# gmongaras/Stable-Diffusion-3-From-Scratch

Measured on AMD Instinct MI355X. Metric: train images/sec MMDiT-B 256^2 bf16, higher is better.
Workload: dtype bf16

## Files before the change

stable-diffusion-3-from-scratch_amd/_lib.py:

```python
import ctypes
import os
import re

_HERE = os.path.dirname(os.path.abspath(__file__))
def experiment(name: str, default: str) -> str:
    return os.environ.get(name, default) if os.environ.get("MMDIT_EXPERIMENTS") == "1" else default


LIB_PATH = os.environ.get("MMDIT_LIB") or os.path.join(_HERE, "libmmdit_hip.so")
HEADER_PATH = os.path.join(_HERE, "..", "include", "mmdit_hip.h")
HEADER_EXT_PATH = os.path.join(_HERE, "..", "include", "mmdit_hip_ext.h")

F32, BF16 = 0, 1
ACT_NONE, ACT_SILU, ACT_SWIGLU, ACT_SWIGLU_BWD = 0, 1, 2, 3
PREC_BF16, PREC_SPLIT = 0, 1
FP8 = 2

_vp, _i, _i64, _f, _d = ctypes.c_void_p, ctypes.c_int, ctypes.c_int64, ctypes.c_float, ctypes.c_double


class GemmArgs(ctypes.Structure):
    _fields_ = [
        ("A", _vp), ("a_dtype", _i), ("a_kmajor", _i), ("lda", _i64),
        ("B", _vp), ("b_dtype", _i), ("b_kmajor", _i), ("ldb", _i64),
        ("C", _vp), ("c_dtype", _i), ("ldc", _i64),
        ("M", _i), ("N", _i), ("K", _i),
# ... 22 lines not shown
class LnBwdProblem(ctypes.Structure):
    _fields_ = [("dout", ctypes.c_void_p), ("x", ctypes.c_void_p), ("mean", ctypes.c_void_p), ("rstd", ctypes.c_void_p), ("scale", ctypes.c_void_p),
                ("ld_mod", ctypes.c_int64), ("dres", ctypes.c_void_p), ("rows", ctypes.c_int), ("rows_per_batch", ctypes.c_int),
                ("dx", ctypes.c_void_p), ("dscale", ctypes.c_void_p), ("dshift", ctypes.c_void_p), ("ld_dmod", ctypes.c_int64),
                ("acc", ctypes.c_void_p), ("gate", ctypes.c_void_p), ("ld_gate", ctypes.c_int64), ("dacc", ctypes.c_void_p), ("dgate", ctypes.c_void_p),
                ("ld_dgate", ctypes.c_int64), ("dbias", ctypes.c_void_p), ("ld_dbias", ctypes.c_int64)]


class QkProblem(ctypes.Structure):
    _fields_ = [("qkv", ctypes.c_void_p), ("wq", ctypes.c_void_p), ("wk", ctypes.c_void_p), ("rope_cos", ctypes.c_void_p), ("rope_sin", ctypes.c_void_p),
                ("tokens", ctypes.c_int), ("tok0", ctypes.c_int), ("dqkv", ctypes.c_void_p), ("dwq", ctypes.c_void_p), ("dwk", ctypes.c_void_p)]


class MlpBwdProblem(ctypes.Structure):
    _fields_ = [("dh", ctypes.c_void_p), ("gu", ctypes.c_void_p), ("dgu", ctypes.c_void_p), ("rows", ctypes.c_int), ("dbias", ctypes.c_void_p)]


class QkEpilogue(ctypes.Structure):
    _fields_ = [("wq", _vp), ("wk", _vp), ("rope_cos", _vp), ("rope_sin", _vp), ("tokens", _i), ("tok0", _i)]


_SIGNATURES = {
    "mmdit_abi_version": ([], _i),
    "mmdit_struct_size": ([_i], _i),
    "mmdit_build_arch": ([], ctypes.c_char_p),
    "mmdit_gemm": ([ctypes.POINTER(GemmArgs), _vp], _i),
    "mmdit_gemm_grouped": ([ctypes.POINTER(GemmArgs), _i, _vp], _i),
    "mmdit_gemm_plan": ([ctypes.POINTER(GemmArgs), _i], _i),
    "mmdit_gemm_set_workspace": ([_vp, ctypes.c_longlong], _i),
    "mmdit_debug_occupy": ([_i, ctypes.c_longlong, _vp], _i),
# ... 39 lines not shown
    "mmdit_vae_softmax_rows": ([_vp, _i, _i, _i, ctypes.c_float, _vp, _vp], _i),
    "mmdit_vae_attn_fwd": ([_vp, _vp, _vp, _i, _i, _i, _i, _f, _vp, _vp], _i),
    "mmdit_patchify": ([_vp, _i, _i, _i, _i, _i, _vp, _i, _vp], _i),
    "mmdit_unpatchify": ([_vp, _i, _i, _i, _i, _i, _vp, _i, _vp], _i),
    "mmdit_time_embed_fwd": ([_vp, _vp, _vp, _i, _i, _vp, _i, _vp], _i),
    "mmdit_time_embed_bwd": ([_vp, _i, _vp, _vp, _vp, _i, _i, _vp, _vp], _i),
    "mmdit_grad_sumsq": ([_vp, _vp, _vp, _i, _vp, _vp], _i),
    "mmdit_clip_coef": ([_vp, _i, _vp, _f, _vp, _vp], _i),
    "mmdit_adamw_step": ([_vp, _vp, _vp, _i, _vp, _vp, _d, _d, _d, _d, _d, _vp], _i),
    "mmdit_adamw_step_dlr": ([_vp, _vp, _vp, _i, _vp, _vp, _vp, _d, _d, _d, _d, _vp], _i),
    "mmdit_cast_multi": ([_vp, _vp, _vp, _i, _vp], _i),
}
_EXT_SIGNATURES = {
    "mmdit_attn_fwd_e4m3": ([_vp, _vp, _vp, _i, _i, _i, _i, _f, _vp, _vp, _vp, _vp, _vp], _i),
}
ATTN_E4M3_KEY_TILE, ATTN_E4M3_QUERY_TILE = 64, 128
ADAMW_CHUNK = 65536
ABI_VERSION = 10
_STRUCTS = [("mmdit_gemm_args", GemmArgs), ("mmdit_ln_fwd_problem", LnFwdProblem), ("mmdit_ln_bwd_problem", LnBwdProblem),
            ("mmdit_qk_problem", QkProblem), ("mmdit_mlp_bwd_problem", MlpBwdProblem), ("mmdit_adamw_tensor", None), ("mmdit_cast_tensor", None), ("mmdit_qk_epilogue", QkEpilogue)]

_lib = None


def declared_symbols():
    with open(HEADER_PATH) as f:
        txt = f.read()
    return sorted(set(re.findall(r"\b(mmdit_[a-z0-9_]+)\s*\(", txt)) - {"mmdit_stream_t"})


def declared_ext_symbols():
    with open(HEADER_EXT_PATH) as f:
        txt = f.read()
    return sorted(set(re.findall(r"\b(mmdit_[a-z0-9_]+)\s*\(", txt)) - {"mmdit_stream_t"})


def lib():
    global _lib
    if _lib is None:
        if not os.path.exists(LIB_PATH):
            raise RuntimeError(
                f"{LIB_PATH} is missing: build it with `python __graft_entry__.py build` "
                "(hipcc --offload-arch=gfx950).  There is no PyTorch/CPU fallback for the MMDiT hot path.")
        try:
            import torch
            if torch.cuda.is_available():
                torch.cuda.init()
        except ImportError:
            pass
        L = ctypes.CDLL(LIB_PATH)
        for name, (argtypes, restype) in list(_SIGNATURES.items()) + list(_EXT_SIGNATURES.items()):
            fn = getattr(L, name)
            fn.argtypes = argtypes
            fn.restype = restype
        if L.mmdit_abi_version() != ABI_VERSION:
            raise RuntimeError(f"{LIB_PATH}: ABI version {L.mmdit_abi_version()}, this binding is written for {ABI_VERSION}: rebuild (python __graft_entry__.py build)")
        for which, (name, struct) in enumerate(_STRUCTS):
            if struct is not None and L.mmdit_struct_size(which) != ctypes.sizeof(struct):
                raise RuntimeError(f"{LIB_PATH}: sizeof({name}) = {L.mmdit_struct_size(which)}, the binding's ctypes mirror has {ctypes.sizeof(struct)} bytes")
        _lib = L
    return _lib


ERR_ARG, ERR_DTYPE, ERR_SHAPE = -1, -2, -3


# ... 5 lines not shown
```

stable-diffusion-3-from-scratch_amd/build.py:

```python
import hashlib
import os
import subprocess
import sys
from concurrent.futures import ThreadPoolExecutor

HERE = os.path.dirname(os.path.abspath(__file__))
CSRC = os.path.join(HERE, "csrc")
LIB = os.path.join(HERE, "libmmdit_hip.so")
HEADER = os.path.join(HERE, "..", "include", "mmdit_hip.h")
HEADER_EXT = os.path.join(HERE, "..", "include", "mmdit_hip_ext.h")
SOURCES = ["gemm.hip", "gemm_dma.hip", "gemm_lean.hip", "gemm8p.hip", "gemm8p_inf.hip", "rowops.hip", "attention.hip", "attention_e4m3.hip", "vae.hip", "vae_attn.hip", "optim.hip"]
HIPCC = os.environ.get("HIPCC", "/opt/rocm/bin/hipcc")
FLAGS = ["--offload-arch=gfx950", "-O3", "-std=c++17", "-fPIC"] + os.environ.get("MMDIT_EXTRA_HIPCC_FLAGS", "").split()
SOURCE_FLAGS = {"vae_attn.hip": ["-mllvm", "-amdgpu-mfma-vgpr-form=1"]}


def _sha(paths, extra=""):
    h = hashlib.sha256(extra.encode())
    for p in paths:
        with open(p, "rb") as f:
            h.update(os.path.basename(p).encode() + b"\0" + f.read() + b"\0")
    return h.hexdigest()


def _read(path):
    try:
        with open(path) as f:
            return f.read().strip()
    except OSError:
        return None


def source_hash(src):
    headers = sorted(os.path.join(CSRC, f) for f in os.listdir(CSRC) if f.endswith(".h")) + [HEADER, HEADER_EXT]
    if src == "gemm8p_inf.hip":
        headers.append(os.path.join(CSRC, "gemm8p.hip"))
    return _sha([os.path.join(CSRC, src)] + headers, " ".join([HIPCC] + FLAGS + SOURCE_FLAGS.get(src, [])))


def build(force: bool = False, verbose: bool = False) -> str:
    want = {src: source_hash(src) for src in SOURCES}

    def cc(src):
        obj = os.path.join(CSRC, src.replace(".hip", ".o"))
        if not force and os.path.exists(obj) and _read(obj + ".sha") == want[src]:
            return obj, False
        cmd = [HIPCC] + FLAGS + SOURCE_FLAGS.get(src, []) + ["-c", os.path.join(CSRC, src), "-o", obj]
        if verbose:
            print(" ".join(cmd), flush=True)
# ... 27 lines not shown
```

stable-diffusion-3-from-scratch_amd/csrc/rowops.hip:

```cpp
#include "common.h"
#include <float.h>

namespace {

constexpr float LN_EPS = 1e-5f;
constexpr float RMS_EPS = FLT_EPSILON;

__device__ __forceinline__ float bf16_round(float x) { return __builtin_bit_cast(float, pack_bf2(x, 0.f) << 16); }

template <int NITX, typename TO, typename TA, bool RES, bool MX = false>
__device__ __forceinline__ void ln_mod_fwd_body(int block, const float* __restrict__ x, const float* __restrict__ scale, const float* __restrict__ shift,
                                                int64_t ld_mod, int rows, int d, int rpb, TO* __restrict__ out,
                                                float* __restrict__ mean_o, float* __restrict__ rstd_o,
                                                const TA* __restrict__ acc, const float* __restrict__ gate, int64_t ld_gate, float* __restrict__ xo,
                                                unsigned char* __restrict__ mx_scales) {
  constexpr int NIT = NITX < 0 ? -NITX : NITX;
  constexpr bool EXACT = NITX < 0;
  const int lane = threadIdx.x & 63, row = block * 4 + (threadIdx.x >> 6);
  if (row >= rows) return;
  const int nch = d >> 2;
  const int b = row / rpb;
  const float* xr = x + (int64_t)row * d;
  float v[NIT][4];
  float s = 0.f;
// ... 865 lines not shown
  __syncthreads();
  if (rl == 0 && c < cols && dbias) dbias[(int64_t)blockIdx.y * cols + c] += sb[0][cl] + sb[1][cl] + sb[2][cl] + sb[3][cl];
}

template <typename TI, typename TO>
__global__ void cast_kernel(const TI* __restrict__ src, TO* __restrict__ dst, int64_t n) {
  const int64_t n8 = n >> 3;
  for (int64_t i = (int64_t)blockIdx.x * blockDim.x + threadIdx.x; i < n8; i += (int64_t)gridDim.x * blockDim.x) {
    float v[8];
    ld8(src + i * 8, v);
    st8(dst + i * 8, v);
  }
  if (blockIdx.x == 0 && threadIdx.x < (n & 7)) io<TO>::st(dst + n8 * 8 + threadIdx.x, io<TI>::ld(src + n8 * 8 + threadIdx.x));
}

template <typename TI, typename TO, bool TO_TOKENS>
__global__ void patch_kernel(const TI* __restrict__ src, TO* __restrict__ dst, int batch, int ch, int H, int W) {
  const int W2 = W >> 1, H2 = H >> 1;
  const int64_t total = (int64_t)batch * ch * H * W2;
  for (int64_t g = (int64_t)blockIdx.x * blockDim.x + threadIdx.x; g < total; g += (int64_t)gridDim.x * blockDim.x) {
    const int j = (int)(g % W2); int64_t r = g / W2;
    const int y = (int)(r % H); r /= H;
    const int c = (int)(r % ch); const int64_t b = r / ch;
    const int64_t img_off = ((b * ch + c) * H + y) * W + 2 * j;
    const int64_t tok_off = ((b * H2 + (y >> 1)) * W2 + j) * (int64_t)(ch * 4) + c * 4 + (y & 1) * 2;
    if (TO_TOKENS) { io<TO>::st(dst + tok_off, io<TI>::ld(src + img_off)); io<TO>::st(dst + tok_off + 1, io<TI>::ld(src + img_off + 1)); }
    else { io<TO>::st(dst + img_off, io<TI>::ld(src + tok_off)); io<TO>::st(dst + img_off + 1, io<TI>::ld(src + tok_off + 1)); }
  }
}

// ... 592 lines not shown
  else if (x_dtype == MMDIT_BF16) hipLaunchKernelGGL((fp8_quant_kernel<bf16_t>), grid, dim3(256), 0, s, (const bf16_t*)x, n / 8, amax, (uint2*)q_fp8, scale);
  else return MMDIT_ERR_DTYPE;
  return mmdit_launch_status();
}

extern "C" int mmdit_cast(const void* src, int src_dtype, void* dst, int dst_dtype, int64_t n, mmdit_stream_t stream) {
  MMDIT_CHECK_ARG(src && dst && n > 0);
  hipStream_t s = (hipStream_t)stream;
  dim3 grid(grid_cap(n / 8 + 1, 256));
  if (src_dtype == MMDIT_F32 && dst_dtype == MMDIT_BF16) hipLaunchKernelGGL((cast_kernel<float, bf16_t>), grid, dim3(256), 0, s, (const float*)src, (bf16_t*)dst, n);
  else if (src_dtype == MMDIT_BF16 && dst_dtype == MMDIT_F32) hipLaunchKernelGGL((cast_kernel<bf16_t, float>), grid, dim3(256), 0, s, (const bf16_t*)src, (float*)dst, n);
  else return MMDIT_ERR_DTYPE;
  return mmdit_launch_status();
}

template <bool TO_TOKENS>
static int patch_dispatch(const void* src, int sdt, void* dst, int ddt, int batch, int ch, int H, int W, mmdit_stream_t stream) {
  MMDIT_CHECK_ARG(src && dst && batch > 0 && ch > 0 && H > 0 && W > 0 && H % 2 == 0 && W % 2 == 0);
  hipStream_t s = (hipStream_t)stream;
  dim3 grid(grid_cap((int64_t)batch * ch * H * (W / 2), 256));
#define PK(TI, TO) hipLaunchKernelGGL((patch_kernel<TI, TO, TO_TOKENS>), grid, dim3(256), 0, s, (const TI*)src, (TO*)dst, batch, ch, H, W)
  if (sdt == MMDIT_F32 && ddt == MMDIT_F32) PK(float, float);
  else if (sdt == MMDIT_F32 && ddt == MMDIT_BF16) PK(float, bf16_t);
  else if (sdt == MMDIT_BF16 && ddt == MMDIT_BF16) PK(bf16_t, bf16_t);
  else if (sdt == MMDIT_BF16 && ddt == MMDIT_F32) PK(bf16_t, float);
  else return MMDIT_ERR_DTYPE;
#undef PK
  return mmdit_launch_status();
}
extern "C" int mmdit_patchify(const void* img, int img_dtype, int batch, int ch, int H, int W, void* tokens, int tok_dtype, mmdit_stream_t st) {
// ... 24 lines not shown
```

stable-diffusion-3-from-scratch_amd/engine.py:

```python
from types import SimpleNamespace as NS

import torch

from . import _lib, ops
from ._lib import ACT_SILU, PREC_BF16, PREC_SPLIT

F32 = torch.float32
BF16 = torch.bfloat16


class Mode:
    def __init__(self, fast: bool = True, fp8: bool = False, mx: bool = False):
        self.fast = fast
        self.fp8 = fp8
        self.mx = mx
        self.T = BF16 if fast else F32
        self.prec = PREC_BF16 if fast else PREC_SPLIT
        self.attn_mode = 0 if fast else 1
        self.attn_e4m3 = False
        self._q = {}

    def act(self, t):
        return t if t.dtype == self.T else ops.cast(t, self.T)

# ... 336 lines not shown
    else:
        C2 = Pending(sv.C1)
    if not lazy:
        X2, C2 = X2.value(), C2.value()
    return X2, C2, sv


_LN_PAIR = _lib.experiment("MMDIT_LN_PAIR", "1") != "0"
_MX_FUSE = _lib.experiment("MMDIT_MX_FUSE", "1") != "0"
_BATCH_WMOD = _lib.experiment("MMDIT_BATCH_WMOD", "1") != "0"
_QKV_FUSE = _lib.experiment("MMDIT_QKV_FUSE", "1") != "0"
_QKV_RAW = _lib.experiment("MMDIT_QKV_RAW", "0") == "1"
_QK_FUSE = _lib.experiment("MMDIT_ATTN_QK_FUSE", "1") != "0"
_FUSE_SWIGLU_BWD = _lib.experiment("MMDIT_FUSE_SWIGLU_BWD", "1") != "0"
_FUSE_GATE = _lib.experiment("MMDIT_FUSE_GATE", "1") != "0"


def _qk_bwd_two_pass(m, w, sv, g, dOx, dOc, dims, rope, dev):
    B, N, Mt, H, d = dims
    S = N + Mt
    if w.kv_merge:
        dQ, dK, dV = ops.attn_bwd(sv.Q, sv.K, sv.V, sv.Ox, sv.Oc, dOx, dOc, sv.lse, N, 64 ** -0.5, m.T, s_kv=S // 2)
        return ops.qk_norm_rope_bwd_merge_pair(dQ, dK, dV, (sv.qkv_x, w.wq_x, w.wk_x, rope[0], rope[1], N, 0, g.wq_x, g.wk_x),
                                               (sv.qkv_c, w.wq_c, w.wk_c, None, None, Mt, N, g.wq_c, g.wk_c), B, H, S, m.T)
    dQ, dK, dV = ops.attn_bwd(sv.Q, sv.K, sv.V, sv.Ox, sv.Oc, dOx, dOc, sv.lse, N, 64 ** -0.5, m.T)
    if _LN_PAIR and dev.type == "cuda":
        return ops.qk_norm_rope_bwd_pair(dQ, dK, dV, (sv.qkv_x, w.wq_x, w.wk_x, rope[0], rope[1], N, 0, g.wq_x, g.wk_x),
                                         (sv.qkv_c, w.wq_c, w.wk_c, None, None, Mt, N, g.wq_c, g.wk_c), B, H, S, m.T)
    dqkv_x = ops.qk_norm_rope_bwd(dQ, dK, dV, sv.qkv_x, w.wq_x, w.wk_x, rope[0], rope[1], B, N, H, S, 0, g.wq_x, g.wk_x, m.T)
    dqkv_c = ops.qk_norm_rope_bwd(dQ, dK, dV, sv.qkv_c, w.wq_c, w.wk_c, None, None, B, Mt, H, S, N, g.wq_c, g.wk_c, m.T)
# ... 4 lines not shown
    B, N, Mt, H, d = dims
    both = not w.last
    ms = _mod_views(sv.mod, d, w.last)
    g = NS(mlp_x=NS(), mlp_c=NS() if both else None)
    hx = sv.gu_x.shape[1]
    nb = 2 if both else 1
    shapes = [(nb * d,), (hx,), (64,), (64,), (64,), (64,)] + ([(sv.gu_c.shape[1],)] if both else []) + ([] if defer_cond else [(d,)])
    npar = len(shapes)
    shapes += [tuple(sv.mod.shape), (B, nb * d)]
    zs, small_arena = _zeros_views(shapes, dev, prefix=npar)
    st = NS(g=g, ms=ms, zs=zs, npar=npar, small_arena=small_arena, both=both)
    st.bdown, g.mlp_x.bup, g.wq_x, g.wk_x, g.wq_c, g.wk_c = zs[:6]
    if not defer_cond:
        g.by = zs[npar - 1]
    st.dmod, st.bpart = zs[npar], zs[npar + 1]
    g.mlp_x.bdown = st.bdown[:d]
    if both:
        g.mlp_c.bdown, g.mlp_c.bup = st.bdown[d:], zs[6]
    st.dms = _mod_views(st.dmod, d, w.last)
    st.req_x = (sv.acc_mx, ms.gate2x, st.dms.gate2x, st.bpart[:, :d])
    st.req_c = (sv.acc_mc, ms.gate2c, st.dms.gate2c, st.bpart[:, d:]) if both else None
    return st


def block_bwd(m, w, sv, dX2, dC2, dy_acc, dims, rope, defer_cond=False, st=None, dacc=None, nxt=None, defer_wmod=False):
    B, N, Mt, H, d = dims
    S, dev = N + Mt, dX2.device
    both = not w.last
    if st is None:
        st = block_bwd_begin(m, w, sv, dims, dev, defer_cond)
    g, ms, dms, bpart, bdown, dmod = st.g, st.ms, st.dms, st.bpart, st.bdown, st.dmod
    pending = []
    fuse = _FUSE_GATE

    def defer(ns, name, dY, Xa):
        pending.append((lambda o, ns=ns, name=name: setattr(ns, name, o), _wg(dY, Xa)))

    dacc_x = dacc[0] if dacc is not None else ops.gate_residual_bwd(dX2, sv.acc_mx, ms.gate2x, N, dms.gate2x, bpart[:, :d], m.T)
    probs = [dict(A=dacc_x, B=w.mlp_x.Wdown, b_kmajor=True, out_dtype=m.T)]
    if both:
        dacc_c = dacc[1] if dacc is not None else ops.gate_residual_bwd(dC2, sv.acc_mc, ms.gate2c, Mt, dms.gate2c, bpart[:, d:], m.T)
        probs.append(dict(A=dacc_c, B=w.mlp_c.Wdown, b_kmajor=True, out_dtype=m.T))
    ops.colsum(bpart, bdown)
    dgu = None
    if (_FUSE_SWIGLU_BWD and m.fast and dev.type == "cuda" and m.prec == PREC_BF16 and dacc_x.dtype == BF16 and sv.gu_x.dtype == BF16
            and not w.mlp_x.gelu and (not both or not w.mlp_c.gelu)):
        fp = [dict(A=dacc_x, B=w.mlp_x.Wdown, aux=sv.gu_x, dbias=g.mlp_x.bup, precision=m.prec)]
        if both:
            fp.append(dict(A=dacc_c, B=w.mlp_c.Wdown, aux=sv.gu_c, dbias=g.mlp_c.bup, precision=m.prec))
        dgu = ops.gemm_swiglu_bwd(fp)
    if dgu is None:
        dh = _group(m, probs)
    defer(g.mlp_x, "Wdown", dacc_x, sv.h_x)
    pair = both and _LN_PAIR and dev.type == "cuda" and w.mlp_x.hidden == w.mlp_c.hidden and w.mlp_x.gelu == w.mlp_c.gelu
    if dgu is not None:
        dgu_x, dgu_c = dgu[0], (dgu[1] if both else None)
    elif pair:
        dgu_x, dgu_c = ops.mlp_act_bwd_pair((dh[0], sv.gu_x, g.mlp_x.bup), (dh[1], sv.gu_c, g.mlp_c.bup), w.mlp_x.hidden, w.mlp_x.gelu)
# ... 44 lines not shown
    else:
        dqkv_x, dqkv_c = _qk_bwd_two_pass(m, w, sv, g, dOx, dOc, dims, rope, dev)
    dln1 = _group(m, [dict(A=dqkv_x, B=w.Wqkv_x, b_kmajor=True, out_dtype=m.T), dict(A=dqkv_c, B=w.Wqkv_c, b_kmajor=True, out_dtype=m.T)])
    defer(g, "Wqkv_x", dqkv_x, sv.ln1x)
    defer(g, "Wqkv_c", dqkv_c, sv.ln1c)
    nacc = None
    ax = dict(dout=dln1[0], x=sv.X, mean=sv.mu1x, rstd=sv.rs1x, scale=ms.scale1x, dres=dX1, rpb=N, dscale=dms.scale1x, dshift=dms.shift1x)
    ac = dict(dout=dln1[1], x=sv.C, mean=sv.mu1c, rstd=sv.rs1c, scale=ms.scale1c, dres=dC1, rpb=Mt, dscale=dms.scale1c, dshift=dms.shift1c)
    if nxt is not None and fuse:
        ax["gated"], ac["gated"] = nxt.req_x, nxt.req_c
        (dX, nax), (dC, nac) = _ln_bwd_pair(ax, ac)
        nacc = (nax, nac)
    else:
        dX, dC = _ln_bwd_pair(ax, ac)

    dmod_a = m.act(dmod)
    if defer_cond:
        if not defer_wmod:
            defer(g, "Wmod", dmod_a, sv.yp)
        dy_acc = dmod_a
    else:
        defer(g, "Wmod", dmod_a, sv.yp)
        dyp = _dgrad(m, dmod_a, w.Wmod, F32, **({"split_k": 16} if m.fast else {}))
        dpre = ops.silu_bwd(dyp, sv.pre, m.T, g.by)
        dy_acc = _dgrad(m, dpre, w.Wy, F32, residual=dy_acc)
        defer(g, "Wy", dpre, sv.y)

    wg_arena = _wgrad_flush(m, pending)
    g.arenas = [wg_arena, st.small_arena] if wg_arena is not None else None
    if nxt is not None:
        return dX, dC, dy_acc, g, nacc
# ... 48 lines not shown
        elif torch.is_tensor(v):
            out.append(v)
    return out


def _set_grad_tensors(g, new, pos=0):
    for k, v in list(vars(g).items()):
        if isinstance(v, NS):
            pos = _set_grad_tensors(v, new, pos)
        elif torch.is_tensor(v):
            setattr(g, k, new[pos])
            pos += 1
    return pos


def model_bwd(m, W, sv, dv, rope, on_grads=None):
    B, N, Mt, H, d = sv.dims
    _, Cin, Hh, Ww = sv.img
    dev = dv.device
    if dev.type == "cuda":
        ops.zero_pool_begin(dev)
    g = NS()
    pending = []

    def defer(name, dY, Xa):
        pending.append((lambda o, name=name: setattr(g, name, o), _wg(dY, Xa)))

    dZ = ops.patchify(dv.contiguous(), m.T)
    g.bout = ops.zeros(W.Wout.shape[0], dev)
    ops.colsum(dZ, g.bout)
    dlnf = _dgrad(m, dZ, W.Wout, m.T)
    defer("Wout", dZ, sv.lnf)
    dmodo = ops.zeros(sv.modo.shape, dev) if sv.modo.dtype == F32 else torch.zeros_like(sv.modo)
    nblk = len(W.blocks)
    sts = [None] * nblk
    sts[nblk - 1] = block_bwd_begin(m, W.blocks[-1], sv.blocks[-1], sv.dims, dev, defer_cond=True)
    dacc = None
    if _FUSE_GATE:
        dX, dax = ops.ln_modulate_bwd(dlnf, sv.Xf, sv.muf, sv.rsf, sv.modo[:, d:], None, N, dmodo[:, d:], dmodo[:, :d], gated=sts[-1].req_x)
        dacc = (dax, None)
    else:
        dX = ops.ln_modulate_bwd(dlnf, sv.Xf, sv.muf, sv.rsf, sv.modo[:, d:], None, N, dmodo[:, d:], dmodo[:, :d])
    dmodo_a = m.act(dmodo)
    dy_acc = _dgrad(m, dmodo_a, W.Wmod_out, F32, **({"split_k": 4} if m.fast else {}))
    defer("Wmod_out", dmodo_a, sv.y)

    dC = None
    g.blocks = [None] * nblk
    dmods = [None] * nblk
    yps = [None] * nblk
    batch_wmod = on_grads is None and _BATCH_WMOD
    for i in range(nblk - 1, -1, -1):
        if i > 0:
            sts[i - 1] = block_bwd_begin(m, W.blocks[i - 1], sv.blocks[i - 1], sv.dims, dev, defer_cond=True)
            dX, dC, dmods[i], g.blocks[i], dacc = block_bwd(m, W.blocks[i], sv.blocks[i], dX, dC, None, sv.dims, rope, defer_cond=True,
                                                            st=sts[i], dacc=dacc, nxt=sts[i - 1], defer_wmod=batch_wmod)
        else:
            dX, dC, dmods[i], g.blocks[i] = block_bwd(m, W.blocks[i], sv.blocks[i], dX, dC, None, sv.dims, rope, defer_cond=True, st=sts[i], dacc=dacc,
                                                      defer_wmod=batch_wmod)
        sts[i] = None
        yps[i] = sv.blocks[i].yp
        sv.blocks[i] = None
        if on_grads is not None:
            repl = on_grads(_grad_tensors(g.blocks[i]), _wg_streams.get(dev), g.blocks[i].arenas)
            if repl is not None:
                _set_grad_tensors(g.blocks[i], repl)

    dyp_all = ops.zeros((nblk * B, d), dev)
    by_all = ops.zeros((nblk, d), dev)
    for i0 in range(0, nblk, 12):
        _group(m, [dict(A=dmods[i], B=W.blocks[i].Wmod, b_kmajor=True, out=dyp_all[i * B:(i + 1) * B], **({"split_k": 4} if m.fast else {}))
                   for i in range(i0, min(nblk, i0 + 12))])
    dpre_all = ops.silu_bwd(dyp_all, sv.pre_all, m.T, by_all, rows_per_bias=B)
    dyc = torch.empty((nblk + 1, B, d), dtype=F32, device=dev)
    dyc[nblk].copy_(dy_acc)
    for i0 in range(0, nblk, 12):
        _group(m, [dict(A=dpre_all[i * B:(i + 1) * B], B=W.blocks[i].Wy, b_kmajor=True, out=dyc[i]) for i in range(i0, min(nblk, i0 + 12))])
    dy_acc = dyc.sum(0)
    late = []
    for i in range(nblk):
        g.blocks[i].by = by_all[i]
        pending.append((lambda o, i=i: setattr(g.blocks[i], "Wy", o), _wg(dpre_all[i * B:(i + 1) * B], sv.y)))
        late += [(i, "by"), (i, "Wy")]
        if batch_wmod:
            pending.append((lambda o, i=i: setattr(g.blocks[i], "Wmod", o), _wg(dmods[i], yps[i])))

    g.bpe = ops.zeros(d, dev)
    ops.colsum(dX, g.bpe)
    dX_a = m.act(dX)
    dX0 = _dgrad(m, dX_a, W.Wpe, m.T)
    defer("Wpe", dX_a, sv.X0)
    defer("Wpatch", dX0, sv.patches)

    dCv = dC.view(B, Mt, d)
    dc1 = m.act(dCv[:, :W.split].reshape(B * W.split, d))
    dc2 = m.act(dCv[:, W.split:].reshape(B * (Mt - W.split), d))
    dcn1, dcn2 = _group(m, [dict(A=dc1, B=W.Wc1, b_kmajor=True, out_dtype=m.T), dict(A=dc2, B=W.Wc2, b_kmajor=True, out_dtype=m.T)])
    defer("Wc1", dc1, sv.cn1)
    defer("Wc2", dc2, sv.cn2)
    g.wn1, g.wn2, g.s1, g.s2 = ops.text_rmsnorm_bwd(dcn1, dcn2, sv.c, W.wn1, W.wn2, W.s1, W.s2, W.split)

    dy_a = m.act(dy_acc)
    defer("Wcond", dy_a, sv.cp)
    dpe = _dgrad(m, dy_a, W.Wt, m.T)
    defer("Wt", dy_a, sv.pe)
    g.time_scale = ops.time_embed_bwd(dpe, sv.t, W.time_scale, W.denom)
    _wgrad_flush(m, pending)
    if on_grads is not None:
        keys = [k for k, v in vars(g).items() if torch.is_tensor(v)]
        repl = on_grads([getattr(g, k) for k in keys] + [getattr(g.blocks[i], n) for i, n in late], _wg_streams.get(dev))
        if repl is not None:
# ... 7 lines not shown
```

stable-diffusion-3-from-scratch_amd/model_trainer.py:

```python
import copy
import json
import math
import os
import time

import torch
import torch.distributed as dist
from torch import nn

from .helpers.multi_gpu_helpers import is_main_process
from .helpers.TimeSampler import TimeSampler
from .helpers.checkpoint_stream import CheckpointStreamer
from .helpers.wire_format import unpad_latents
from .optim import ClipAdamW
from .reducer import GradReducer, broadcast_parameters


def get_scheduler(optimizer, num_warmup_steps, num_training_steps, use_lr_scheduler):
    if use_lr_scheduler:
        def lr_lambda(step):
            if step < num_warmup_steps:
                return float(step) / float(max(1, num_warmup_steps))
            progress = float(step - num_warmup_steps) / float(max(1, num_training_steps - num_warmup_steps))
            return max(0.0, 0.5 * (1.0 + math.cos(math.pi * 0.5 * 2.0 * progress)))
# ... 300 lines not shown
        return loss

    def can_capture(self):
        if self.device.type != "cuda" or not self.hip_optimizer:
            return "needs hip_optimizer=True on a GPU"
        if self.ema_model_cpu is not None and self._ema_gpu is None:
            return "the EMA must live on the GPU (ema_on_gpu=True) or be off"
        if self.reducer.enabled and dist.get_backend(self.subgroup) != "nccl":
            return "the gradient collectives are captured with the step: backend nccl (RCCL) only"
        return None

    def capture_graph(self, step):
        why = self.can_capture()
        if why is not None:
            raise RuntimeError("capture_graph: " + why)
        from . import engine
        if engine._WG_OVERLAP:
            engine._WG_OVERLAP = False
        in_graph = isinstance(self.data_source, SyntheticData) and self.device_rng
        self._slots = None
        if not in_graph:
            self._slots = [tuple(x.to(self.device).clone() for x in self._draw()) for _ in range(self.accumulation_steps)]
        torch.cuda.synchronize(self.device)
        if self.reducer.enabled and self.device.type == "cuda":
            self.capture_handoff = "polled" if self._wait_for_watchdog() else "heuristic"
        self.optim.sync_lr(self.device)
        self.optim.prepare_capture()
        self._loss_out = torch.zeros((), dtype=torch.float32, device=self.device)
        g = torch.cuda.CUDAGraph(keep_graph=True) if self.keep_graph else torch.cuda.CUDAGraph()
        for gen in (self._gen, getattr(self.data_source, "g", None)) if in_graph else ():
            if gen is not None:
                g.register_generator_state(gen)
        self.optim.zero_grad()
        try:
            with torch.cuda.graph(g, capture_error_mode="thread_local" if self.reducer.enabled else "global"):
                loss = None
                for k in range(self.accumulation_steps):
                    l = self.micro_step(final=(k == self.accumulation_steps - 1), inputs=None if in_graph else self._slots[k])
                    loss = l if loss is None else loss + l
                self._hip_optimizer_step()
                if self.grad_scaler is not None:
                    self.grad_scaler.update()
# ... 317 lines not shown
```

stable-diffusion-3-from-scratch_amd/ops.py:

```python
import ctypes
import os

import torch

from . import _lib
from ._lib import ACT_NONE, ACT_SILU, ACT_SWIGLU, ACT_SWIGLU_BWD, BF16, F32, FP8, PREC_BF16, PREC_SPLIT, GemmArgs, check

_DT = {torch.float32: F32, torch.bfloat16: BF16, torch.float8_e4m3fn: FP8}

PROFILE = None
_ZERO_ALL = _lib.experiment("MMDIT_ZERO_ALL", "0") == "1"


class _ZeroPool:

    def __init__(self):
        self.buf, self.off, self.cap, self.need = None, 0, 0, 0

    def begin(self, device):
        self.cap = max(self.cap, self.need)
        self.need, self.off = 0, 0
        self.buf = torch.zeros(self.cap, dtype=torch.float32, device=device) if self.cap else None

    def take(self, numel, device):
# ... 671 lines not shown
    if v.dtype != torch.float32 or x0.dtype != eps.dtype or x0.numel() != n or eps.numel() != n or n % 8:
        raise RuntimeError("flow_loss: v fp32, x0 and eps of one dtype and v's size, numel % 8 == 0")
    loss = torch.empty((), dtype=torch.float32, device=v.device)
    part = torch.empty(256, dtype=torch.float32, device=v.device)
    dv = torch.empty(v.shape, dtype=torch.float32, device=v.device) if need_grad else None
    check(_lib.lib().mmdit_flow_loss(_p(_c(v)), _p(_c(x0)), _p(_c(eps)), _dt(x0), n, 1.0 / (n * accumulation_steps), _p(dv), _p(part), _p(loss), _s()), "mmdit_flow_loss")
    return loss, dv


def colsum(x, out):
    rows, cols = x.shape
    check(_lib.lib().mmdit_colsum(_p(x), _dt(x), rows, cols, x.stride(0), _p(out), _s()), "mmdit_colsum")
    return out


def patchify(img, out_dtype):
    batch, ch, H, W = img.shape
    tokens = torch.empty((batch * (H // 2) * (W // 2), ch * 4), dtype=out_dtype, device=img.device)
    check(_lib.lib().mmdit_patchify(_p(_c(img)), _dt(img), batch, ch, H, W, _p(tokens), _dt(tokens), _s()), "mmdit_patchify")
    return tokens


def unpatchify(tokens, batch, ch, H, W, out_dtype):
    img = torch.empty((batch, ch, H, W), dtype=out_dtype, device=tokens.device)
    check(_lib.lib().mmdit_unpatchify(_p(_c(tokens)), _dt(tokens), batch, ch, H, W, _p(img), _dt(img), _s()), "mmdit_unpatchify")
    return img


def time_embed_fwd(t, time_scale, denom, out_dtype):
    batch, dim = t.shape[0], denom.shape[0]
# ... 76 lines not shown
```

Before: 2349.

## Add grouped backward-finish kernel fusing column sums and bf16 casts

```diff
diff --git a/include/mmdit_hip_train.h b/include/mmdit_hip_train.h
--- /dev/null
+++ b/include/mmdit_hip_train.h
@@ -0,0 +1,28 @@
+#ifndef MMDIT_HIP_TRAIN_H
+#define MMDIT_HIP_TRAIN_H
+
+#include "mmdit_hip.h"
+
+#ifdef __cplusplus
+extern "C" {
+#endif
+
+#define MMDIT_FINISH_MAX_PROBLEMS 64
+#define MMDIT_FINISH_TABLE_BYTES 8192
+
+typedef struct {
+  const void* x;
+  int x_dtype;
+  int groups, rows, cols;
+  int64_t ld, group_stride;
+  float* sum_out;
+  void* cast_out;
+} mmdit_finish_problem;
+
+int mmdit_backward_finish(const mmdit_finish_problem* probs, int count, void* table_dev, void* staging_host, mmdit_stream_t stream);
+
+#ifdef __cplusplus
+}
+#endif
+
+#endif
diff --git a/stable-diffusion-3-from-scratch_amd/_lib.py b/stable-diffusion-3-from-scratch_amd/_lib.py
--- a/stable-diffusion-3-from-scratch_amd/_lib.py
+++ b/stable-diffusion-3-from-scratch_amd/_lib.py
@@ -10,6 +10,7 @@
 LIB_PATH = os.environ.get("MMDIT_LIB") or os.path.join(_HERE, "libmmdit_hip.so")
 HEADER_PATH = os.path.join(_HERE, "..", "include", "mmdit_hip.h")
 HEADER_EXT_PATH = os.path.join(_HERE, "..", "include", "mmdit_hip_ext.h")
+HEADER_TRAIN_PATH = os.path.join(_HERE, "..", "include", "mmdit_hip_train.h")
 
 F32, BF16 = 0, 1
 ACT_NONE, ACT_SILU, ACT_SWIGLU, ACT_SWIGLU_BWD = 0, 1, 2, 3
@@ -62,6 +63,11 @@
 
 class MlpBwdProblem(ctypes.Structure):
     _fields_ = [("dh", ctypes.c_void_p), ("gu", ctypes.c_void_p), ("dgu", ctypes.c_void_p), ("rows", ctypes.c_int), ("dbias", ctypes.c_void_p)]
+
+
+class FinishProblem(ctypes.Structure):
+    _fields_ = [("x", ctypes.c_void_p), ("x_dtype", ctypes.c_int), ("groups", ctypes.c_int), ("rows", ctypes.c_int), ("cols", ctypes.c_int),
+                ("ld", ctypes.c_int64), ("group_stride", ctypes.c_int64), ("sum_out", ctypes.c_void_p), ("cast_out", ctypes.c_void_p)]
 
 
 class QkEpilogue(ctypes.Structure):
@@ -131,6 +137,10 @@
 _EXT_SIGNATURES = {
     "mmdit_attn_fwd_e4m3": ([_vp, _vp, _vp, _i, _i, _i, _i, _f, _vp, _vp, _vp, _vp, _vp], _i),
 }
+_TRAIN_SIGNATURES = {
+    "mmdit_backward_finish": ([ctypes.POINTER(FinishProblem), _i, _vp, _vp, _vp], _i),
+}
+FINISH_MAX_PROBLEMS, FINISH_TABLE_BYTES = 64, 8192
 ATTN_E4M3_KEY_TILE, ATTN_E4M3_QUERY_TILE = 64, 128
 ADAMW_CHUNK = 65536
 ABI_VERSION = 10
@@ -148,6 +158,12 @@
 
 def declared_ext_symbols():
     with open(HEADER_EXT_PATH) as f:
+        txt = f.read()
+    return sorted(set(re.findall(r"\b(mmdit_[a-z0-9_]+)\s*\(", txt)) - {"mmdit_stream_t"})
+
+
+def declared_train_symbols():
+    with open(HEADER_TRAIN_PATH) as f:
         txt = f.read()
     return sorted(set(re.findall(r"\b(mmdit_[a-z0-9_]+)\s*\(", txt)) - {"mmdit_stream_t"})
 
@@ -166,7 +182,7 @@
         except ImportError:
             pass
         L = ctypes.CDLL(LIB_PATH)
-        for name, (argtypes, restype) in list(_SIGNATURES.items()) + list(_EXT_SIGNATURES.items()):
+        for name, (argtypes, restype) in list(_SIGNATURES.items()) + list(_EXT_SIGNATURES.items()) + list(_TRAIN_SIGNATURES.items()):
             fn = getattr(L, name)
             fn.argtypes = argtypes
             fn.restype = restype
diff --git a/stable-diffusion-3-from-scratch_amd/build.py b/stable-diffusion-3-from-scratch_amd/build.py
--- a/stable-diffusion-3-from-scratch_amd/build.py
+++ b/stable-diffusion-3-from-scratch_amd/build.py
@@ -9,6 +9,7 @@
 LIB = os.path.join(HERE, "libmmdit_hip.so")
 HEADER = os.path.join(HERE, "..", "include", "mmdit_hip.h")
 HEADER_EXT = os.path.join(HERE, "..", "include", "mmdit_hip_ext.h")
+HEADER_TRAIN = os.path.join(HERE, "..", "include", "mmdit_hip_train.h")
 SOURCES = ["gemm.hip", "gemm_dma.hip", "gemm_lean.hip", "gemm8p.hip", "gemm8p_inf.hip", "rowops.hip", "attention.hip", "attention_e4m3.hip", "vae.hip", "vae_attn.hip", "optim.hip"]
 HIPCC = os.environ.get("HIPCC", "/opt/rocm/bin/hipcc")
 FLAGS = ["--offload-arch=gfx950", "-O3", "-std=c++17", "-fPIC"] + os.environ.get("MMDIT_EXTRA_HIPCC_FLAGS", "").split()
@@ -32,7 +33,7 @@
 
 
 def source_hash(src):
-    headers = sorted(os.path.join(CSRC, f) for f in os.listdir(CSRC) if f.endswith(".h")) + [HEADER, HEADER_EXT]
+    headers = sorted(os.path.join(CSRC, f) for f in os.listdir(CSRC) if f.endswith(".h")) + [HEADER, HEADER_EXT, HEADER_TRAIN]
     if src == "gemm8p_inf.hip":
         headers.append(os.path.join(CSRC, "gemm8p.hip"))
     return _sha([os.path.join(CSRC, src)] + headers, " ".join([HIPCC] + FLAGS + SOURCE_FLAGS.get(src, [])))
diff --git a/stable-diffusion-3-from-scratch_amd/csrc/rowops.hip b/stable-diffusion-3-from-scratch_amd/csrc/rowops.hip
--- a/stable-diffusion-3-from-scratch_amd/csrc/rowops.hip
+++ b/stable-diffusion-3-from-scratch_amd/csrc/rowops.hip
@@ -1,5 +1,7 @@
 #include "common.h"
+#include "../../include/mmdit_hip_train.h"
 #include <float.h>
+#include <string.h>
 
 namespace {
 
@@ -903,6 +905,68 @@
   if (blockIdx.x == 0 && threadIdx.x < (n & 7)) io<TO>::st(dst + n8 * 8 + threadIdx.x, io<TI>::ld(src + n8 * 8 + threadIdx.x));
 }
 
+struct FinProb {
+  const void* x; float* out; bf16_t* y;
+  int64_t ld, gs;
+  int rows, cols, f32, lc;
+  int rpt, nslab, nchunk, wg0;
+};
+struct FinTable { int wg_end[MMDIT_FINISH_MAX_PROBLEMS]; FinProb p[MMDIT_FINISH_MAX_PROBLEMS]; };
+static_assert(sizeof(FinTable) <= MMDIT_FINISH_TABLE_BYTES, "the finish table must fit the buffers the header promises");
+
+template <typename T>
+__device__ __forceinline__ void finish_body(const FinProb& p, int local, float* sbuf ) {
+  const int lc = p.lc, c = 1 << lc, nrl = 256 >> lc;
+  const int tx = threadIdx.x & (c - 1), rl = threadIdx.x >> lc;
+  const int slab = local % p.nslab, rest = local / p.nslab, chunk = rest % p.nchunk, g = rest / p.nchunk;
+  const int col = ((slab << lc) + tx) * 8;
+  const int rbeg = chunk * nrl * p.rpt, rend = min(p.rows, rbeg + nrl * p.rpt);
+  float s[8];
+#pragma unroll
+  for (int e = 0; e < 8; e++) s[e] = 0.f;
+  if (col < p.cols) {
+    const T* xb = (const T*)p.x + (int64_t)g * p.gs + col;
+    bf16_t* yb = p.y ? p.y + (int64_t)g * p.rows * p.cols + col : nullptr;
+    for (int r0 = rbeg + rl; r0 < rend; r0 += 4 * nrl) {
+      float v[4][8];
+#pragma unroll
+      for (int k = 0; k < 4; k++) ld8(xb + (int64_t)min(r0 + k * nrl, rend - 1) * p.ld, v[k]);
+#pragma unroll
+      for (int k = 0; k < 4; k++) {
+        const int r = r0 + k * nrl;
+        if (r < rend) {
+#pragma unroll
+          for (int e = 0; e < 8; e++) s[e] += v[k][e];
+          if (yb) st8(yb + (int64_t)r * p.cols, v[k]);
+        }
+      }
+    }
+  }
+  if (p.out) {
+    const int w = c * 8;
+    st8(sbuf + rl * w + tx * 8, s);
+    __syncthreads();
+    for (int j = threadIdx.x; j < w; j += 256) {
+      const int cc = (slab << lc) * 8 + j;
+      if (cc < p.cols) {
+        float t = 0.f;
+        for (int q = 0; q < nrl; q++) t += sbuf[q * w + j];
+        atomicAdd(p.out + cc, t);
+      }
+    }
+  }
+}
+
+__global__ __launch_bounds__(256) void backward_finish_kernel(const FinTable* __restrict__ tab, int count) {
+  __shared__ float sbuf[2048];
+  const int bid = blockIdx.x;
+  int pi = 0;
+  while (pi < count - 1 && bid >= tab->wg_end[pi]) pi++;
+  const FinProb p = tab->p[pi];
+  if (p.f32) finish_body<float>(p, bid - p.wg0, sbuf);
+  else finish_body<bf16_t>(p, bid - p.wg0, sbuf);
+}
+
 template <typename TI, typename TO, bool TO_TOKENS>
 __global__ void patch_kernel(const TI* __restrict__ src, TO* __restrict__ dst, int batch, int ch, int H, int W) {
   const int W2 = W >> 1, H2 = H >> 1;
@@ -1525,6 +1589,40 @@
   return mmdit_launch_status();
 }
 
+extern "C" int mmdit_backward_finish(const mmdit_finish_problem* probs, int count, void* table_dev, void* staging_host, mmdit_stream_t stream) {
+  MMDIT_CHECK_ARG(probs && table_dev && staging_host && count >= 1 && count <= MMDIT_FINISH_MAX_PROBLEMS && (uintptr_t)table_dev % 16 == 0);
+  FinTable t;
+  memset(&t, 0, sizeof(t));
+  int64_t wg = 0;
+  for (int i = 0; i < count; i++) {
+    const mmdit_finish_problem& q = probs[i];
+    MMDIT_CHECK_ARG(q.x && (q.sum_out || q.cast_out) && q.groups > 0 && q.rows > 0 && q.cols > 0 && q.cols % 8 == 0 && q.ld >= q.cols && q.ld % 8 == 0 &&
+                    q.group_stride >= 0 && q.group_stride % 8 == 0);
+    MMDIT_CHECK_ARG((uintptr_t)q.x % 16 == 0 && (uintptr_t)q.sum_out % 16 == 0 && (uintptr_t)q.cast_out % 16 == 0);
+    if (q.x_dtype != MMDIT_F32 && q.x_dtype != MMDIT_BF16) return MMDIT_ERR_DTYPE;
+    const bool flat = q.groups == 1 || (q.group_stride == (int64_t)q.rows * q.ld && (int64_t)q.groups * q.rows <= (1 << 30));
+    const int groups = flat ? 1 : q.groups, rows = flat ? q.groups * q.rows : q.rows;
+    if (rows > (1 << 30)) return MMDIT_ERR_SHAPE;
+    const int cp = q.cols / 8;
+    int lc = 8;
+    while (lc > 0 && (int64_t)((cp + (1 << lc) - 1) >> lc << lc) * 100 > (int64_t)cp * 115) lc--;
+    const int nrl = 256 >> lc;
+    const int64_t bytes = (int64_t)q.groups * q.rows * q.cols * (q.x_dtype == MMDIT_F32 ? 4 : 2);
+    const int rpt = bytes >= (16ll << 20) ? 8 : 4;
+    const int nslab = (cp + (1 << lc) - 1) >> lc, nchunk = (rows + nrl * rpt - 1) / (nrl * rpt);
+    t.p[i] = FinProb{q.x, q.sum_out, (bf16_t*)q.cast_out, q.ld, q.group_stride, rows, q.cols, q.x_dtype == MMDIT_F32, lc, rpt, nslab, nchunk, (int)wg};
+    wg += (int64_t)groups * nchunk * nslab;
+    if (wg > (1ll << 30)) return MMDIT_ERR_SHAPE;
+    t.wg_end[i] = (int)wg;
+  }
+  hipStream_t s = (hipStream_t)stream;
+  memcpy(staging_host, &t, sizeof(t));
+  hipError_t e = hipMemcpyAsync(table_dev, staging_host, sizeof(t), hipMemcpyHostToDevice, s);
+  if (e != hipSuccess) return (int)e;
+  hipLaunchKernelGGL(backward_finish_kernel, dim3((unsigned)wg), dim3(256), 0, s, (const FinTable*)table_dev, count);
+  return mmdit_launch_status();
+}
+
 template <bool TO_TOKENS>
 static int patch_dispatch(const void* src, int sdt, void* dst, int ddt, int batch, int ch, int H, int W, mmdit_stream_t stream) {
   MMDIT_CHECK_ARG(src && dst && batch > 0 && ch > 0 && H > 0 && W > 0 && H % 2 == 0 && W % 2 == 0);
diff --git a/stable-diffusion-3-from-scratch_amd/engine.py b/stable-diffusion-3-from-scratch_amd/engine.py
--- a/stable-diffusion-3-from-scratch_amd/engine.py
+++ b/stable-diffusion-3-from-scratch_amd/engine.py
@@ -374,6 +374,8 @@
 _QK_FUSE = _lib.experiment("MMDIT_ATTN_QK_FUSE", "1") != "0"
 _FUSE_SWIGLU_BWD = _lib.experiment("MMDIT_FUSE_SWIGLU_BWD", "1") != "0"
 _FUSE_GATE = _lib.experiment("MMDIT_FUSE_GATE", "1") != "0"
+_FINISH_FOLD = _lib.experiment("MMDIT_FINISH_FOLD", "0") == "1"
+_BIAS_DIRECT = _lib.experiment("MMDIT_BIAS_DIRECT", "0") == "1"
 
 
 def _qk_bwd_two_pass(m, w, sv, g, dOx, dOc, dims, rope, dev):
@@ -408,6 +410,9 @@
     if not defer_cond:
         g.by = zs[npar - 1]
     st.dmod, st.bpart = zs[npar], zs[npar + 1]
+    st.direct = _BIAS_DIRECT and dev.type == "cuda"
+    if st.direct:
+        st.bpart = st.bdown.unsqueeze(0).expand(B, nb * d)
     g.mlp_x.bdown = st.bdown[:d]
     if both:
         g.mlp_c.bdown, g.mlp_c.bup = st.bdown[d:], zs[6]
@@ -417,9 +422,10 @@
     return st
 
 
-def block_bwd(m, w, sv, dX2, dC2, dy_acc, dims, rope, defer_cond=False, st=None, dacc=None, nxt=None, defer_wmod=False):
+def block_bwd(m, w, sv, dX2, dC2, dy_acc, dims, rope, defer_cond=False, st=None, dacc=None, nxt=None, defer_wmod=False, defer_finish=False):
     B, N, Mt, H, d = dims
     S, dev = N + Mt, dX2.device
+    assert not defer_finish or (defer_cond and defer_wmod and st is not None)
     both = not w.last
     if st is None:
         st = block_bwd_begin(m, w, sv, dims, dev, defer_cond)
@@ -435,7 +441,8 @@
     if both:
         dacc_c = dacc[1] if dacc is not None else ops.gate_residual_bwd(dC2, sv.acc_mc, ms.gate2c, Mt, dms.gate2c, bpart[:, d:], m.T)
         probs.append(dict(A=dacc_c, B=w.mlp_c.Wdown, b_kmajor=True, out_dtype=m.T))
-    ops.colsum(bpart, bdown)
+    if not defer_finish and not st.direct:
+        ops.colsum(bpart, bdown)
     dgu = None
     if (_FUSE_SWIGLU_BWD and m.fast and dev.type == "cuda" and m.prec == PREC_BF16 and dacc_x.dtype == BF16 and sv.gu_x.dtype == BF16
             and not w.mlp_x.gelu and (not both or not w.mlp_c.gelu)):
@@ -510,7 +517,7 @@
     else:
         dX, dC = _ln_bwd_pair(ax, ac)
 
-    dmod_a = m.act(dmod)
+    dmod_a = dmod if defer_finish else m.act(dmod)
     if defer_cond:
         if not defer_wmod:
             defer(g, "Wmod", dmod_a, sv.yp)
@@ -589,6 +596,10 @@
     return pos
 
 
+def finish_launches(nblk):
+    return 1 + (2 * nblk + 4 + _lib.FINISH_MAX_PROBLEMS - 1) // _lib.FINISH_MAX_PROBLEMS
+
+
 def model_bwd(m, W, sv, dv, rope, on_grads=None):
     B, N, Mt, H, d = sv.dims
     _, Cin, Hh, Ww = sv.img
@@ -603,7 +614,12 @@
 
     dZ = ops.patchify(dv.contiguous(), m.T)
     g.bout = ops.zeros(W.Wout.shape[0], dev)
-    ops.colsum(dZ, g.bout)
+    finish = m.fast and dev.type == "cuda" and m.T == BF16
+    fold = finish and _FINISH_FOLD
+    if finish:
+        ops.backward_finish([(dZ, g.bout, None)])
+    else:
+        ops.colsum(dZ, g.bout)
     dlnf = _dgrad(m, dZ, W.Wout, m.T)
     defer("Wout", dZ, sv.lnf)
     dmodo = ops.zeros(sv.modo.shape, dev) if sv.modo.dtype == F32 else torch.zeros_like(sv.modo)
@@ -616,23 +632,28 @@
         dacc = (dax, None)
     else:
         dX = ops.ln_modulate_bwd(dlnf, sv.Xf, sv.muf, sv.rsf, sv.modo[:, d:], None, N, dmodo[:, d:], dmodo[:, :d])
-    dmodo_a = m.act(dmodo)
-    dy_acc = _dgrad(m, dmodo_a, W.Wmod_out, F32, **({"split_k": 4} if m.fast else {}))
-    defer("Wmod_out", dmodo_a, sv.y)
+    if not fold:
+        dmodo_a = m.act(dmodo)
+        dy_acc = _dgrad(m, dmodo_a, W.Wmod_out, F32, **({"split_k": 4} if m.fast else {}))
+        defer("Wmod_out", dmodo_a, sv.y)
 
     dC = None
     g.blocks = [None] * nblk
     dmods = [None] * nblk
     yps = [None] * nblk
     batch_wmod = on_grads is None and _BATCH_WMOD
+    fin_blocks = fold and batch_wmod
+    fin = []
     for i in range(nblk - 1, -1, -1):
         if i > 0:
             sts[i - 1] = block_bwd_begin(m, W.blocks[i - 1], sv.blocks[i - 1], sv.dims, dev, defer_cond=True)
             dX, dC, dmods[i], g.blocks[i], dacc = block_bwd(m, W.blocks[i], sv.blocks[i], dX, dC, None, sv.dims, rope, defer_cond=True,
-                                                            st=sts[i], dacc=dacc, nxt=sts[i - 1], defer_wmod=batch_wmod)
+                                                            st=sts[i], dacc=dacc, nxt=sts[i - 1], defer_wmod=batch_wmod, defer_finish=fin_blocks)
         else:
             dX, dC, dmods[i], g.blocks[i] = block_bwd(m, W.blocks[i], sv.blocks[i], dX, dC, None, sv.dims, rope, defer_cond=True, st=sts[i], dacc=dacc,
-                                                      defer_wmod=batch_wmod)
+                                                      defer_wmod=batch_wmod, defer_finish=fin_blocks)
+        if fin_blocks and not sts[i].direct:
+            fin.append((sts[i].bpart, sts[i].bdown, None))
         sts[i] = None
         yps[i] = sv.blocks[i].yp
         sv.blocks[i] = None
@@ -641,14 +662,41 @@
             if repl is not None:
                 _set_grad_tensors(g.blocks[i], repl)
 
+    dyc = torch.empty((nblk + 1, B, d), dtype=F32, device=dev)
+    if finish:
+        if fin_blocks:
+            stack = torch.empty(sum(t.numel() for t in dmods), dtype=BF16, device=dev)
+            off = 0
+            for i in range(nblk):
+                a = stack[off:off + dmods[i].numel()].view(dmods[i].shape)
+                off += dmods[i].numel()
+                fin.append((dmods[i], None, a))
+                dmods[i] = a
+        g.bpe = ops.zeros(d, dev)
+        dX_a = torch.empty((B * N, d), dtype=BF16, device=dev)
+        fin.append((dX, g.bpe, dX_a))
+        if fold:
+            dCv = dC.view(B, Mt, d)
+            dc1 = torch.empty((B * W.split, d), dtype=BF16, device=dev)
+            dc2 = torch.empty((B * (Mt - W.split), d), dtype=BF16, device=dev)
+            dmodo_a = torch.empty(dmodo.shape, dtype=BF16, device=dev)
+            fin += [(dCv[:, :W.split], None, dc1), (dCv[:, W.split:], None, dc2), (dmodo, None, dmodo_a)]
+        ops.backward_finish(fin)
+        fin = None
+    if fold:
+        head = dyc[nblk]
+        head._mmdit_zero_check = True
+        _dgrad(m, dmodo_a, W.Wmod_out, F32, out=head, split_k=4)
+        defer("Wmod_out", dmodo_a, sv.y)
+
     dyp_all = ops.zeros((nblk * B, d), dev)
     by_all = ops.zeros((nblk, d), dev)
     for i0 in range(0, nblk, 12):
         _group(m, [dict(A=dmods[i], B=W.blocks[i].Wmod, b_kmajor=True, out=dyp_all[i * B:(i + 1) * B], **({"split_k": 4} if m.fast else {}))
                    for i in range(i0, min(nblk, i0 + 12))])
     dpre_all = ops.silu_bwd(dyp_all, sv.pre_all, m.T, by_all, rows_per_bias=B)
-    dyc = torch.empty((nblk + 1, B, d), dtype=F32, device=dev)
-    dyc[nblk].copy_(dy_acc)
+    if not fold:
+        dyc[nblk].copy_(dy_acc)
     for i0 in range(0, nblk, 12):
         _group(m, [dict(A=dpre_all[i * B:(i + 1) * B], B=W.blocks[i].Wy, b_kmajor=True, out=dyc[i]) for i in range(i0, min(nblk, i0 + 12))])
     dy_acc = dyc.sum(0)
@@ -660,16 +708,18 @@
         if batch_wmod:
             pending.append((lambda o, i=i: setattr(g.blocks[i], "Wmod", o), _wg(dmods[i], yps[i])))
 
-    g.bpe = ops.zeros(d, dev)
-    ops.colsum(dX, g.bpe)
-    dX_a = m.act(dX)
+    if not finish:
+        g.bpe = ops.zeros(d, dev)
+        ops.colsum(dX, g.bpe)
+        dX_a = m.act(dX)
     dX0 = _dgrad(m, dX_a, W.Wpe, m.T)
     defer("Wpe", dX_a, sv.X0)
     defer("Wpatch", dX0, sv.patches)
 
-    dCv = dC.view(B, Mt, d)
-    dc1 = m.act(dCv[:, :W.split].reshape(B * W.split, d))
-    dc2 = m.act(dCv[:, W.split:].reshape(B * (Mt - W.split), d))
+    if not fold:
+        dCv = dC.view(B, Mt, d)
+        dc1 = m.act(dCv[:, :W.split].reshape(B * W.split, d))
+        dc2 = m.act(dCv[:, W.split:].reshape(B * (Mt - W.split), d))
     dcn1, dcn2 = _group(m, [dict(A=dc1, B=W.Wc1, b_kmajor=True, out_dtype=m.T), dict(A=dc2, B=W.Wc2, b_kmajor=True, out_dtype=m.T)])
     defer("Wc1", dc1, sv.cn1)
     defer("Wc2", dc2, sv.cn2)
diff --git a/stable-diffusion-3-from-scratch_amd/model_trainer.py b/stable-diffusion-3-from-scratch_amd/model_trainer.py
--- a/stable-diffusion-3-from-scratch_amd/model_trainer.py
+++ b/stable-diffusion-3-from-scratch_amd/model_trainer.py
@@ -338,7 +338,7 @@
         why = self.can_capture()
         if why is not None:
             raise RuntimeError("capture_graph: " + why)
-        from . import engine
+        from . import engine, ops
         if engine._WG_OVERLAP:
             engine._WG_OVERLAP = False
         in_graph = isinstance(self.data_source, SyntheticData) and self.device_rng
@@ -350,6 +350,7 @@
             self.capture_handoff = "polled" if self._wait_for_watchdog() else "heuristic"
         self.optim.sync_lr(self.device)
         self.optim.prepare_capture()
+        self._finish_staging = ops.finish_prepare_capture(self.accumulation_steps * engine.finish_launches(len(self.model.blocks)))
         self._loss_out = torch.zeros((), dtype=torch.float32, device=self.device)
         g = torch.cuda.CUDAGraph(keep_graph=True) if self.keep_graph else torch.cuda.CUDAGraph()
         for gen in (self._gen, getattr(self.data_source, "g", None)) if in_graph else ():
diff --git a/stable-diffusion-3-from-scratch_amd/ops.py b/stable-diffusion-3-from-scratch_amd/ops.py
--- a/stable-diffusion-3-from-scratch_amd/ops.py
+++ b/stable-diffusion-3-from-scratch_amd/ops.py
@@ -709,6 +709,53 @@
     return out
 
 
+_FIN_RING = {}
+_FIN_CAPTURE = None
+
+
+def finish_prepare_capture(launches):
+    global _FIN_CAPTURE
+    bufs = [torch.empty(_lib.FINISH_TABLE_BYTES, dtype=torch.uint8).pin_memory() for _ in range(int(launches))]
+    _FIN_CAPTURE = dict(bufs=bufs, next=0)
+    return bufs
+
+
+def backward_finish(items):
+    L = _lib.lib()
+    dev = items[0][0].device
+    for i0 in range(0, len(items), _lib.FINISH_MAX_PROBLEMS):
+        part = items[i0:i0 + _lib.FINISH_MAX_PROBLEMS]
+        arr = (_lib.FinishProblem * len(part))()
+        for q, (x, sum_out, cast_out) in zip(arr, part):
+            if x.dim() not in (2, 3) or x.stride(-1) != 1 or (sum_out is not None and (sum_out.dtype != torch.float32 or sum_out.numel() != x.shape[-1] or not sum_out.is_contiguous())) \
+                    or (cast_out is not None and (cast_out.dtype != torch.bfloat16 or cast_out.numel() != x.numel() or not cast_out.is_contiguous())):
+                raise RuntimeError("backward_finish: x (rows, cols) or (groups, rows, cols) with unit inner stride, sum_out fp32 (cols,), cast_out contiguous bf16 of x's size")
+            q.x, q.x_dtype, q.sum_out, q.cast_out = _p(x), _dt(x), _p(sum_out), _p(cast_out)
+            q.groups, q.rows, q.cols = (x.shape[0] if x.dim() == 3 else 1), x.shape[-2], x.shape[-1]
+            q.ld, q.group_stride = x.stride(-2), (x.stride(0) if x.dim() == 3 else 0)
+        event = None
+        if torch.cuda.is_current_stream_capturing():
+            c = _FIN_CAPTURE
+            if c is None or c["next"] >= len(c["bufs"]):
+                raise RuntimeError("backward_finish: call finish_prepare_capture() before capturing a step into a graph")
+            staging = c["bufs"][c["next"]]
+            c["next"] += 1
+        else:
+            ring = _FIN_RING.get(dev)
+            if ring is None:
+                ring = _FIN_RING[dev] = dict(bufs=[torch.empty(_lib.FINISH_TABLE_BYTES, dtype=torch.uint8).pin_memory() for _ in range(8)], events=[None] * 8, slot=0)
+            slot = ring["slot"]
+            ring["slot"] = (slot + 1) % 8
+            if ring["events"][slot] is not None:
+                ring["events"][slot].synchronize()
+            staging = ring["bufs"][slot]
+            event = ring["events"][slot] = torch.cuda.Event()
+        table = torch.empty(_lib.FINISH_TABLE_BYTES, dtype=torch.uint8, device=dev)
+        check(L.mmdit_backward_finish(arr, len(part), _p(table), staging.data_ptr(), _s()), "mmdit_backward_finish")
+        if event is not None:
+            event.record(torch.cuda.current_stream(dev))
+
+
 def patchify(img, out_dtype):
     batch, ch, H, W = img.shape
     tokens = torch.empty((batch * (H // 2) * (W // 2), ch * 4), dtype=out_dtype, device=img.device)
```

After: 2356 (median of 6 runs). No clear change (+0.3%).
